# AlejandroSilvestri/os1

Hardware: AMD Instinct MI355X
Metric: frames/sec extract+match, 1920x1080 @ 2000 ORB feats (higher is better)
Workload: dtype u8

## Files before the change

os1_amd/csrc/orbfe_extractor.hip:

```cpp
#include <hip/hip_runtime.h>
#include <unistd.h>
#include <sched.h>

#include <algorithm>
#include <cctype>
#include <chrono>
#include <cmath>
#include <cstdarg>
#include <cstdio>
#include <cstdlib>
#include <cstring>
#include <memory>
#include <mutex>
#include <string>
#include <thread>
#include <vector>

#include "../../include/orbfe.h"
#include "glibc_sincosf.h"
#include "host_pool.h"
#include "orbfe_internal.h"
#include "quadtree.h"

namespace orbfe {
// ... 292 lines not shown
    Q.minTh = minTh;
    long long off = 0, slot = 0;
    int cellBase = 0;
    size_t tableBytes = 0;
    for (int l = 0; l < nlevels; l++) {
      LevelGeom& L = Q.lv[l];
      L.w = cv_round_f((float)c * isf[l]);
      L.h = cv_round_f((float)r * isf[l]);
      const float width = (float)((L.w - kEdge + 3) - (kEdge - 3));
      const float height = (float)((L.h - kEdge + 3) - (kEdge - 3));
      L.nCols = (int)(width / 30.f);
      L.nRows = (int)(height / 30.f);
      if (L.nCols < 1 || L.nRows < 1) {
        set_err("image %dx%d too small: level %d (%dx%d) has no FAST cell", c, r, l, L.w, L.h);
        return ORBFE_ERR_TOO_SMALL;
      }
      L.wCell = (int)std::ceil(width / L.nCols);
      L.hCell = (int)std::ceil(height / L.nRows);
      {
        const int nIni = (int)roundf(static_cast<float>(L.w - 2 * kBorder) / (L.h - 2 * kBorder));
        if (nIni < 1 || nIni > 4) qtOk = false;
        kpSum += std::max(nfeat[l] + 4, 4 * std::max(nIni, 4));
      }
      L.cellBase = cellBase;
      cellBase += L.nCols * L.nRows;
      L.slotCap = (((L.wCell + 1) / 2) * ((L.hCell + 1) / 2) + 3) & ~3;
      L.slotBase = slot;
      slot += (long long)L.nCols * L.nRows * L.slotCap;
      if (l >= 1) {
        L.pitch = (int)align_up(L.w, 64);
        L.off = off;
        off += align_up((long long)L.pitch * L.h, 256);
        tableBytes += align_up(L.w * 4, 16) + align_up(L.w * 4, 16) + align_up(L.h * 4, 16) + align_up(L.h * 4, 16) + align_up(L.h * 4, 16);
      }
    }
    Q.ncells = cellBase;
    Q.slabBytes = off;
    Q.slotsPerFrame = slot;
    Q.candCap = slot;
    if (slot >= (1ll << 24)) qtOk = false;

    std::vector<uint8_t> tab(tableBytes);
    int rc = d_tables.ensure(tableBytes);
    if (rc) return rc;
    size_t cur = 0;
    const int* xofsH[kMaxLevels] = {};
    const int* yofsH[kMaxLevels] = {};
    for (int l = 1; l < nlevels; l++) {
      LevelGeom& L = Q.lv[l];
      const int sw = Q.lv[l - 1].w, sh = Q.lv[l - 1].h, dw = L.w, dh = L.h;
      const double scale_x = 1. / ((double)dw / sw), scale_y = 1. / ((double)dh / sh);
      int* xofs = (int*)(tab.data() + cur);
      xofsH[l] = xofs;
      L.xofs = (const int*)(d_tables.p + cur);
      cur += align_up(dw * 4, 16);
      short* xa = (short*)(tab.data() + cur);
      L.xalpha = (const short*)(d_tables.p + cur);
      cur += align_up(dw * 4, 16);
      int* yofs = (int*)(tab.data() + cur);
      yofsH[l] = yofs;
      L.yofs = (const int*)(d_tables.p + cur);
      cur += align_up(dh * 4, 16);
      short* yb = (short*)(tab.data() + cur);
      L.ybeta = (const short*)(d_tables.p + cur);
      cur += align_up(dh * 4, 16);
      unsigned* yc = (unsigned*)(tab.data() + cur);
// ... 5 lines not shown
        fx -= sx;
        if (sx < 0) { fx = 0; sx = 0; }
        if (sx >= sw - 1) { fx = 0; sx = sw - 1; }
        xofs[dx] = sx;
        xa[2 * dx] = sat_short(cv_round_f((1.f - fx) * 2048));
        xa[2 * dx + 1] = sat_short(cv_round_f(fx * 2048));
      }
      for (int dy = 0; dy < dh; dy++) {
        float fy = (float)((dy + 0.5) * scale_y - 0.5);
        int sy = cv_floor_f(fy);
        fy -= sy;
        yofs[dy] = sy;
        yc[dy] = (unsigned)std::min(std::max(sy, 0), sh - 1) | ((unsigned)std::min(std::max(sy + 1, 0), sh - 1) << 16);
        yb[2 * dy] = sat_short(cv_round_f((1.f - fy) * 2048));
        yb[2 * dy + 1] = sat_short(cv_round_f(fy * 2048));
      }
      for (int dy = dh; dy < (int)align_up(dh, 4); dy++) {
        yc[dy] = yc[dh - 1];
        yb[2 * dy] = yb[2 * (dh - 1)];
        yb[2 * dy + 1] = yb[2 * (dh - 1) + 1];
      }
      int maxW = 1, maxH = 1;
      for (int x0 = 0; x0 < dw; x0 += 64) {
        const int x1 = std::min(x0 + 64, dw) - 1;
        maxW = std::max(maxW, std::min(xofs[x1] + 1, sw - 1) - xofs[x0] + 1);
      }
      for (int y0 = 0; y0 < dh; y0 += 64) {
        const int y1 = std::min(y0 + 64, dh) - 1;
        const int r0 = std::min(std::max(yofs[y0], 0), sh - 1), r1 = std::min(std::max(yofs[y1] + 1, 0), sh - 1);
        maxH = std::max(maxH, r1 - r0 + 1);
      }
      L.rzPitch = (maxW + 3 + 3) & ~3;
      L.rzRows = maxH;
    }
    HIP_TRY(hipMemcpyAsync(d_tables.p, tab.data(), tableBytes, hipMemcpyHostToDevice, stream));
    auto buildCone = [&](int tile, int baseMin, ConeParams& out, DevBuf<ConeRange>& tabBuf, bool& ok) -> int {
      ok = false;
      if (!(nlevels >= 3 && scaleFactor <= 1.5f)) return ORBFE_OK;
      std::vector<ConeRange> coneTab;
      const int top = nlevels - 1;
      if (tile <= 0) {
        tile = 32;
        for (int t = 16; t < 32; t += 2)
          if (((Q.lv[top].w + t - 1) / t) * ((Q.lv[top].h + t - 1) / t) <= 256) { tile = t; break; }
      }
      const int tx = (Q.lv[top].w + tile - 1) / tile, ty = (Q.lv[top].h + tile - 1) / tile;
      coneTab.assign((size_t)(tx + ty) * kMaxLevels, ConeRange{0, 0});
      int maxW[kMaxLevels] = {}, maxH[kMaxLevels] = {};
      for (int b = 0; b < tx + ty; b++) {
        const bool isX = b < tx;
        int lo = (isX ? b : b - tx) * tile, hi = std::min(lo + tile, isX ? Q.lv[top].w : Q.lv[top].h) - 1;
        ConeRange* R = coneTab.data() + (size_t)b * kMaxLevels;
        for (int l = top;; l--) {
          R[l] = ConeRange{lo, hi};
          int& m = isX ? maxW[l] : maxH[l];
          m = std::max(m, hi - lo + 1);
          if (l == 0) break;
          const int dn = isX ? Q.lv[l].w : Q.lv[l].h, sn = isX ? Q.lv[l - 1].w : Q.lv[l - 1].h;
          const int* ofs = isX ? xofsH[l] : yofsH[l];
          const int nlo = lo == 0 ? 0 : std::min(std::max(ofs[lo], 0), sn - 1);
          const int nhi = hi == dn - 1 ? sn - 1 : std::min(std::max(ofs[hi] + 1, 0), sn - 1);
          lo = nlo; hi = nhi;
        }
      }
      for (int base = std::max(0, baseMin); base < top - 1; base++) {
        auto pitchOf = [&](int l) { return (maxW[l] + 3 + 3) & ~3; };
// ... 1726 lines not shown
```

os1_amd/csrc/orbfe_internal.h:

```cpp
#pragma once
#include <cstddef>
#include <cstdint>

#include "equidistant_tan.h"

namespace orbfe {

constexpr int kMaxLevels = 12;
constexpr int kEdge = 19;
constexpr int kBorder = 16;
constexpr int kHalfPatch = 15;
constexpr int kBlurRad = 18;
constexpr int kRawRad = kBlurRad + 3;

struct LevelGeom {
  int w, h;
  int pitch;
  long long off;
  int nCols, nRows;
  int wCell, hCell;
  int cellBase;
  int slotCap;
  long long slotBase;
  const int* xofs;
  const short* xalpha;
  const int* yofs;
  const short* ybeta;
  const unsigned* yofc;
  int rzPitch, rzRows;
};

struct FastCell {
  uint16_t ex0, ey0;
  uint8_t ew, pad0;
  uint8_t eh, level;
  uint32_t cell;
  uint32_t slotOff;
  uint32_t roiOff;
  uint32_t pitch;
  uint8_t wCell, hCell;
  uint16_t pad1;
  uint32_t geo;
};
static_assert(sizeof(FastCell) == 32, "one s_load_dwordx8 per FAST wave");

struct PyramidParams {
  LevelGeom lv[kMaxLevels];
  int nlevels;
  int ncells;
  long long slabBytes;
  long long slotsPerFrame;
  long long candCap;
  const uint8_t* const* frame0;
  const uint8_t* frameInline[2];
  long long stride0;
  uint8_t* slab;
  uint32_t* cellCount;
  uint32_t* slots;
  uint32_t* cand;
  uint32_t* levelStart;
  const FastCell* cells;
  const uint8_t* zeros;
// ... 116 lines not shown
```

os1_amd/csrc/orbfe_kernels.hip:

```cpp
#include <mutex>
#include <hip/hip_runtime.h>

#include <type_traits>

#include "glibc_sincosf.h"
#include "orbfe_internal.h"

namespace orbfe {

__device__ __forceinline__ int m24(int a, int b) { return __mul24(a, b); }
__device__ __forceinline__ unsigned mulu24(unsigned a, unsigned b) {
  unsigned r;
  asm("v_mul_u32_u24 %0, %1, %2" : "=v"(r) : "v"(a), "v"(b));
  return r;
}

constexpr int kRzTile = 64;

__global__ __launch_bounds__(256) void k_resize(PyramidParams P, int level) {
  extern __shared__ __align__(16) uint8_t rz[];
  const LevelGeom& D = P.lv[level];
  const LevelGeom& S = P.lv[level - 1];
  const int f = P.frameBase + blockIdx.z;
  const int tx0 = blockIdx.x * kRzTile, ty0 = blockIdx.y * kRzTile;
  const int tx1 = min(tx0 + kRzTile, D.w) - 1, ty1 = min(ty0 + kRzTile, D.h) - 1;
  const uint8_t* src;
  long long sstride;
  if (level == 1) {
    src = level0_of(P, f);
    sstride = P.stride0;
  } else {
    src = P.slab + (long long)f * P.slabBytes + S.off;
// ... 84 lines not shown
}
__device__ __forceinline__ unsigned mulu24_w1(unsigned b, unsigned hh) {
  unsigned r;
  asm("v_mul_u32_u24_sdwa %0, %1, %2 dst_sel:DWORD dst_unused:UNUSED_PAD src0_sel:DWORD src1_sel:WORD_1" : "=v"(r) : "v"(b), "v"(hh));
  return r;
}

template <int WA, int WB>
__device__ __forceinline__ unsigned mulu24_hh(unsigned a, unsigned b) {
  unsigned r;
  if (WA == 0 && WB == 0) asm("v_mul_u32_u24_sdwa %0, %1, %2 dst_sel:DWORD dst_unused:UNUSED_PAD src0_sel:WORD_0 src1_sel:WORD_0" : "=v"(r) : "v"(a), "v"(b));
  if (WA == 0 && WB == 1) asm("v_mul_u32_u24_sdwa %0, %1, %2 dst_sel:DWORD dst_unused:UNUSED_PAD src0_sel:WORD_0 src1_sel:WORD_1" : "=v"(r) : "v"(a), "v"(b));
  if (WA == 1 && WB == 0) asm("v_mul_u32_u24_sdwa %0, %1, %2 dst_sel:DWORD dst_unused:UNUSED_PAD src0_sel:WORD_1 src1_sel:WORD_0" : "=v"(r) : "v"(a), "v"(b));
  if (WA == 1 && WB == 1) asm("v_mul_u32_u24_sdwa %0, %1, %2 dst_sel:DWORD dst_unused:UNUSED_PAD src0_sel:WORD_1 src1_sel:WORD_1" : "=v"(r) : "v"(a), "v"(b));
  return r;
}

__device__ __forceinline__ int ld32(const void* base, unsigned byteOff) {
  return *reinterpret_cast<const int*>(reinterpret_cast<const char*>(base) + byteOff);
}

__device__ __forceinline__ const uint8_t* uniform_ptr(const uint8_t* p) {
  const uintptr_t v = reinterpret_cast<uintptr_t>(p);
  const unsigned lo = __builtin_amdgcn_readfirstlane((unsigned)v), hi = __builtin_amdgcn_readfirstlane((unsigned)(v >> 32));
  return reinterpret_cast<const uint8_t*>(((uintptr_t)hi << 32) | lo);
}

__device__ __forceinline__ unsigned pk_round2(unsigned x, unsigned y) {
  unsigned t;
  asm("v_pk_add_u16 %0, %1, %2\n\tv_pk_add_u16 %0, %0, 2 op_sel_hi:[1,0]\n\tv_pk_lshrrev_b16 %0, 2, %0 op_sel_hi:[0,1]" : "=&v"(t) : "v"(x), "v"(y));
  return t;
}

struct ResizeLevel {
  int dw, dh, dpitch;
  int sw, sh;
  long long sstride;
  long long doff, soff;
  const int* xofs;
  const short* xalpha;
  const unsigned* yofc;
  const short* ybeta;
  const uint8_t* const* frame0;
  const uint8_t* frameInline[2];
  uint8_t* slab;
  long long slabBytes;
  int frameBase;
  int fromLevel0;
};

template <int LP, int RH>
__global__ __launch_bounds__(256) void k_resize_fixed(ResizeLevel R, int tilesX, int ntiles, unsigned rcpTilesX, int dma) {
  __shared__ __align__(16) uint8_t rz[LP * RH];
  __shared__ __align__(16) uint16_t H[RH * 64];
  struct { int w, h, pitch; const int* xofs; const short* xalpha; const unsigned* yofc; const short* ybeta; } D = {R.dw, R.dh, R.dpitch, R.xofs, R.xalpha, R.yofc, R.ybeta};
  struct { int w, h; } S = {R.sw, R.sh};
  const int f = R.frameBase + blockIdx.y;
  const int chunk = (ntiles + 7) >> 3;
  const int tileIx = (blockIdx.x & 7) * chunk + (blockIdx.x >> 3);
  if (tileIx >= ntiles) return;
  const int tyI = (int)(((unsigned long long)(unsigned)tileIx * rcpTilesX) >> 32);
  const int tx0 = (tileIx - tyI * tilesX) * kRzTile, ty0 = tyI * kRzTile;
  const int tx1 = min(tx0 + kRzTile, D.w) - 1, ty1 = min(ty0 + kRzTile, D.h) - 1;
  const int level = R.fromLevel0 ? 1 : 2;
  typedef uint32_t u32x2 __attribute__((ext_vector_type(2)));
  u32x2 fpw = {0u, 0u};
  if (R.fromLevel0) {
    if (R.frame0) {
      fpw = *reinterpret_cast<const u32x2 __attribute__((address_space(4)))*>(reinterpret_cast<uintptr_t>(R.frame0 + f));
    } else {
      const unsigned long long v = reinterpret_cast<unsigned long long>((f & 1) ? R.frameInline[1] : R.frameInline[0]);
      fpw.x = (uint32_t)v;
      fpw.y = (uint32_t)(v >> 32);
    }
  }
  const int cxa = *reinterpret_cast<const int __attribute__((address_space(4)))*>(reinterpret_cast<uintptr_t>(D.xofs + tx0));
  const int cxb = *reinterpret_cast<const int __attribute__((address_space(4)))*>(reinterpret_cast<uintptr_t>(D.xofs + tx1));
  const unsigned cya = *reinterpret_cast<const unsigned __attribute__((address_space(4)))*>(reinterpret_cast<uintptr_t>(D.yofc + ty0));
  const unsigned cyb = *reinterpret_cast<const unsigned __attribute__((address_space(4)))*>(reinterpret_cast<uintptr_t>(D.yofc + ty1));
  const int tid = threadIdx.x;
  const int hc = tid & 63;
  const int hx = min(tx0 + hc, D.w - 1);
  const int hsx = ld32(D.xofs, (unsigned)hx << 2);
  const int hal = ld32(D.xalpha, (unsigned)hx << 2);
  const int cx = tx0 + (tid & 15) * 4, cy = ty0 + (tid >> 4) * 4;
  const int4 syq = *reinterpret_cast<const int4*>(reinterpret_cast<const char*>(D.yofc) + ((unsigned)cy << 2));
  const int4 beq = *reinterpret_cast<const int4*>(reinterpret_cast<const char*>(D.ybeta) + ((unsigned)cy << 2));
  const int syv[4] = {syq.x, syq.y, syq.z, syq.w}, be[4] = {beq.x, beq.y, beq.z, beq.w};
  asm volatile("" ::"s"(cxa), "s"(cxb), "s"(cya), "s"(cyb), "s"(fpw.x), "s"(fpw.y));
  const uint8_t* src;
  const long long sstride = R.sstride;
  if (R.fromLevel0) {
    src = reinterpret_cast<const uint8_t*>(((unsigned long long)fpw.y << 32) | fpw.x);
  } else {
    src = R.slab + (long long)f * R.slabBytes + R.soff;
  }
  const int rx0 = cxa, rx1 = min(cxb + 1, S.w - 1);
  const int ry0 = (int)(cya & 0xffffu), ry1 = (int)(cyb >> 16);
  const int rw = rx1 - rx0 + 1, rh = ry1 - ry0 + 1;
  const int istr = (int)sstride;
  const uint8_t* rbase = uniform_ptr(src + (long long)ry0 * sstride + rx0);
  const int a = (int)(reinterpret_cast<uintptr_t>(rbase) & 3);
  if ((sstride & 3) == 0 && dma) {
    static_assert(LP == 96 && RH % 10 == 0, "LDS-DMA staging layout");
    const uint8_t* gb = rbase - a;
    const int lane = tid & 63, wave = __builtin_amdgcn_readfirstlane(tid >> 6);
    const int lrow = (int)(((unsigned)lane * 43u) >> 8), lcol = lane - lrow * 6;
    const bool lastSpecial = level == 1 && ry1 == S.h - 1;
    const int rhDma = lastSpecial ? rh - 1 : rh;
    const bool on = lrow < 10 && 16 * lcol < a + rw;
    const unsigned voff = (unsigned)(m24(lrow, istr) + 16 * lcol);
#pragma unroll
    for (int u = 0; u < RH / 40; u++) {
      const int r = (wave * (RH / 40) + u) * 10;
      const uint8_t* gbr = gb + (long long)r * sstride;
      unsigned vo = voff;
      asm volatile("" : "+s"(gbr), "+v"(vo));
      if (on && r + lrow < rhDma)
        __builtin_amdgcn_global_load_lds((const __attribute__((address_space(1))) void*)(gbr + vo),
                                         (__attribute__((address_space(3))) void*)(rz + r * LP), 16, 0, 0);
    }
    if (lastSpecial && tid < ((a + rw + 3) >> 2))
      *reinterpret_cast<uint32_t*>(rz + (rh - 1) * LP + 4 * tid) = (uint32_t)ld32(gb, (unsigned)(4 * tid + m24(rh - 1, istr)));
    asm volatile("s_waitcnt vmcnt(0)" ::: "memory");
  } else if ((sstride & 3) == 0) {
    static_assert(LP <= 128 && RH % 8 == 0, "staging layout");
    const int ndw = (a + rw + 3) >> 2;
    const int c = tid & 31, r0 = tid >> 5;
    if (c < ndw) {
      const uint8_t* gb = rbase - a;
      uint32_t v[RH / 8];
#pragma unroll
      for (int u = 0; u < RH / 8; u++) v[u] = (uint32_t)ld32(gb, (unsigned)(4 * c + m24(min(r0 + 8 * u, rh - 1), istr)));
      uint8_t* l = rz + 4 * c + r0 * LP;
#pragma unroll
      for (int u = 0; u < RH / 8; u++) *reinterpret_cast<uint32_t*>(l + u * 8 * LP) = v[u];
    }
  } else {
    const float rcp = 1.0f / (float)rw;
    const int total = rw * rh;
    for (int i = tid; i < total; i += 256) {
      const int y = (int)(((float)i + 0.5f) * rcp), x = i - m24(y, rw);
      rz[y * LP + a + x] = rbase[m24(y, istr) + x];
    }
  }
  __syncthreads();
  {
    const unsigned a0 = (unsigned)(int)(short)hal << 12, a1 = (unsigned)(hal >> 16) << 12;
    const int o0 = a + hsx - rx0, o1 = a + min(hsx + 1, S.w - 1) - rx0;
    const uint8_t* p0 = rz + (tid >> 6) * LP + o0;
    const uint8_t* p1 = rz + (tid >> 6) * LP + o1;
    uint16_t* h = H + (tid >> 6) * 64 + hc;
#pragma unroll
    for (int i = 0; i < RH / 4; i++)
      h[i * 4 * 64] = (uint16_t)((__umul24(p0[i * 4 * LP], a0) + __umul24(p1[i * 4 * LP], a1)) >> 16);
  }
  __syncthreads();
  if (cx > tx1 || cy > ty1) return;
  uint8_t* dst = R.slab + (long long)f * R.slabBytes + R.doff;
  unsigned doffs = (unsigned)(m24(cy, D.pitch) + cx);
  const unsigned hx2 = (unsigned)(cx - tx0) * 2u, ry0s = (unsigned)ry0 << 7;
#pragma unroll
  for (int j = 0; j < 4; j++) {
    const int y = cy + j;
    if (y > ty1) break;
    const unsigned r0 = ((unsigned)syv[j] & 0xffffu) << 7, r1 = ((unsigned)syv[j] >> 16) << 7;
    const uint8_t* hb = reinterpret_cast<const uint8_t*>(H) + hx2 - ry0s;
    const uint2 q0 = *reinterpret_cast<const uint2*>(hb + r0), q1 = *reinterpret_cast<const uint2*>(hb + r1);
    const unsigned bw = (unsigned)be[j];
    const unsigned x01 = __builtin_amdgcn_perm(mulu24_hh<0, 1>(bw, q0.x), mulu24_hh<0, 0>(bw, q0.x), 0x07060302u);
    const unsigned y01 = __builtin_amdgcn_perm(mulu24_hh<1, 1>(bw, q1.x), mulu24_hh<1, 0>(bw, q1.x), 0x07060302u);
    const unsigned x23 = __builtin_amdgcn_perm(mulu24_hh<0, 1>(bw, q0.y), mulu24_hh<0, 0>(bw, q0.y), 0x07060302u);
    const unsigned y23 = __builtin_amdgcn_perm(mulu24_hh<1, 1>(bw, q1.y), mulu24_hh<1, 0>(bw, q1.y), 0x07060302u);
    const unsigned v01 = pk_round2(x01, y01), v23 = pk_round2(x23, y23);
    *reinterpret_cast<uint32_t*>(dst + doffs) = __builtin_amdgcn_perm(v23, v01, 0x06040200u);
    doffs += (unsigned)D.pitch;
  }
}

constexpr int kConeThreads = 1024;
#ifdef ORBFE_EXPERIMENTS
__device__ unsigned long long g_coneStamps[32];
#define CONE_STAMP(i)                                                                                                              \
  do {                                                                                                                             \
    if (threadIdx.x == 0 && blockIdx.z == 0 && blockIdx.x == gridDim.x / 2 && blockIdx.y == gridDim.y / 2)                         \
      g_coneStamps[i] = __builtin_amdgcn_s_memrealtime();                                                                          \
  } while (0)
#else
#define CONE_STAMP(i) ((void)0)
#endif

__global__ __launch_bounds__(kConeThreads) void k_pyramid_cone(PyramidParams P, ConeParams C) {
  extern __shared__ __align__(16) uint8_t cone[];
  const int tid = threadIdx.x, f = P.frameBase + blockIdx.z;
// ... 431 lines not shown
  if constexpr (w2 != 0u) acc = __builtin_amdgcn_udot4(d[2], w2, acc, false);
  if constexpr (w3 != 0u) acc = __builtin_amdgcn_udot4(d[3], w3, acc, false);
  return acc;
}

__device__ __forceinline__ int wave_sum_i32(int v) {
  v += __builtin_amdgcn_update_dpp(v, v, 0x128, 0xf, 0xf, false);
  v += __builtin_amdgcn_update_dpp(v, v, 0x124, 0xf, 0xf, false);
  v += __builtin_amdgcn_update_dpp(v, v, 0x122, 0xf, 0xf, false);
  v += __builtin_amdgcn_update_dpp(v, v, 0x121, 0xf, 0xf, false);
  return __builtin_amdgcn_readlane(v, 0) + __builtin_amdgcn_readlane(v, 16) + __builtin_amdgcn_readlane(v, 32) +
         __builtin_amdgcn_readlane(v, 48);
}

__device__ __forceinline__ void wave_sum3_i32(int& a, int& b, int& c) {
#define ORBFE_ROR3(n)                                                          \
  "v_add_u32_dpp %0, %0, %0 row_ror:" #n " row_mask:0xf bank_mask:0xf\n\t"     \
  "v_add_u32_dpp %1, %1, %1 row_ror:" #n " row_mask:0xf bank_mask:0xf\n\t"     \
  "v_add_u32_dpp %2, %2, %2 row_ror:" #n " row_mask:0xf bank_mask:0xf\n\t"
  asm volatile("s_nop 1\n\t" ORBFE_ROR3(8) ORBFE_ROR3(4) ORBFE_ROR3(2) ORBFE_ROR3(1) : "+v"(a), "+v"(b), "+v"(c));
#undef ORBFE_ROR3
  a = __builtin_amdgcn_readlane(a, 0) + __builtin_amdgcn_readlane(a, 16) + __builtin_amdgcn_readlane(a, 32) + __builtin_amdgcn_readlane(a, 48);
  b = __builtin_amdgcn_readlane(b, 0) + __builtin_amdgcn_readlane(b, 16) + __builtin_amdgcn_readlane(b, 32) + __builtin_amdgcn_readlane(b, 48);
  c = __builtin_amdgcn_readlane(c, 0) + __builtin_amdgcn_readlane(c, 16) + __builtin_amdgcn_readlane(c, 32) + __builtin_amdgcn_readlane(c, 48);
}

struct SlotInfo {
  const uint32_t* selCount;
  int selPerFrame;
  int selOff[kMaxLevels + 1];
  int nlevels;
};

struct DescribeLevel { int w, h, pitch, pad; long long off, pad2; };
struct DescribeArgs {
  DescribeLevel lv[kMaxLevels];
  const SelKp* sel;
  const uint32_t* selCount;
  float* angleOut;
  uint8_t* descOut;
  float* angleOut2;
  uint8_t* descOut2;
  const uint8_t* const* frame0;
  const uint8_t* frameInline[2];
  long long stride0;
  uint8_t* slab;
  long long slabBytes;
  int nsel, selPerFrame, nlevels, frameBase, dma;
  int selOff[kMaxLevels + 1];
  int gauss;
};

template <int WAVES, int GAUSS>
__global__ __launch_bounds__(64 * WAVES) void k_describe(DescribeArgs A) {
  constexpr int NT = 64 * WAVES;
  constexpr int NIC = (kIcItems + NT - 1) / NT, NH = (kBlurItemsHost.nh + NT - 1) / NT, NV = (kBlurItemsHost.nv + NT - 1) / NT;
  static_assert(NIC * NT <= 256 && NH * NT <= 512 && NV <= NH, "table padding");
  uint32_t icw[NIC][3], bh[NH], bv[NV];
#pragma unroll
  for (int it = 0; it < NIC; it++) {
    const IcW w = c_icTab.e[it * NT + threadIdx.x];
    icw[it][0] = w.w1; icw[it][1] = w.w2; icw[it][2] = w.w3;
  }
#pragma unroll
  for (int it = 0; it < NH; it++) bh[it] = c_blurCodes.h[it * NT + threadIdx.x];
#pragma unroll
  for (int it = 0; it < NV; it++) bv[it] = c_blurCodes.v[it * NT + threadIdx.x];
  __shared__ int icSum[3 * WAVES];
  __shared__ __align__(16) uint8_t raw[kRawW * kRawP + 16];
  __shared__ __align__(16) uint16_t hbT[40 * kHPT];
  static_assert(kBlurW * kBPT <= kRawW * kRawP, "the blurred patch must fit into the raw patch");
  uint8_t* blT = raw;
  asm volatile("" ::"s"(A.sel), "s"(A.selCount), "s"(A.angleOut), "s"(A.descOut), "s"(A.frame0), "s"(A.frameInline[0]), "s"(A.frameInline[1]),
               "s"(A.stride0), "s"(A.slab), "s"(A.slabBytes), "s"(A.nsel), "s"(A.selPerFrame), "s"(A.nlevels), "s"(A.frameBase), "s"(A.dma),
               "s"(A.selOff[1]), "s"(A.selOff[2]), "s"(A.selOff[3]), "s"(A.selOff[4]), "s"(A.selOff[5]), "s"(A.selOff[6]), "s"(A.selOff[7]));
  const int nsel = A.nsel, dma = A.dma;
  const SelKp* sel = A.sel;
  float* angleOut = A.angleOut;
  uint8_t* descOut = A.descOut;
  const int chunk = (nsel + 7) >> 3;
  const int k = (blockIdx.x & 7) * chunk + (blockIdx.x >> 3);
  if (k >= nsel) return;
  const int tid = threadIdx.x, lane = tid & 63, wave = WAVES == 1 ? 0 : __builtin_amdgcn_readfirstlane(tid >> 6);
  typedef uint32_t u32x2 __attribute__((ext_vector_type(2)));
  typedef uint32_t u32x8 __attribute__((ext_vector_type(8)));
  const char __attribute__((address_space(4)))* ka = (const char __attribute__((address_space(4)))*)__builtin_amdgcn_kernarg_segment_ptr();
  int level, f;
  u32x2 sw, fpw = {0u, 0u};
  u32x8 lw;
  auto frame_ptr_words = [&](int fa) -> u32x2 {
    u32x2 r;
    if (A.frame0) {
      r = *reinterpret_cast<const u32x2 __attribute__((address_space(4)))*>(reinterpret_cast<uintptr_t>(A.frame0 + fa));
    } else {
      const unsigned long long v = reinterpret_cast<unsigned long long>((fa & 1) ? A.frameInline[1] : A.frameInline[0]);
      r.x = (uint32_t)v;
      r.y = (uint32_t)(v >> 32);
    }
    return r;
  };
  if (A.selCount) {
    const int fr = k / A.selPerFrame, within = k - fr * A.selPerFrame;
    int l = 0, lbase = 0;
#pragma unroll
    for (int j = 1; j < kMaxLevels; j++) {
      const int o = A.selOff[j];
      if (j < A.nlevels && within >= o) { l = j; lbase = o; }
    }
    level = l;
    f = A.frameBase + fr;
    const uint32_t live = *reinterpret_cast<const uint32_t __attribute__((address_space(4)))*>(
        reinterpret_cast<uintptr_t>(A.selCount + (long long)f * kMaxLevels + l));
    sw = *reinterpret_cast<const u32x2 __attribute__((address_space(4)))*>(reinterpret_cast<uintptr_t>(sel + k));
    fpw = frame_ptr_words(f);
    lw = *reinterpret_cast<const u32x8 __attribute__((address_space(4)))*>(ka + offsetof(DescribeArgs, lv) + 32 * (unsigned)l);
    asm volatile("" ::"s"(sw.x), "s"(live), "s"(fpw.x), "s"(lw[0]));
    if ((uint32_t)(within - lbase) >= live) return;
  } else {
    sw = *reinterpret_cast<const u32x2 __attribute__((address_space(4)))*>(reinterpret_cast<uintptr_t>(sel + k));
    level = (int)(sw.y & 0xffu);
    f = (int)((sw.y >> 8) & 0xffffu);
    fpw = frame_ptr_words(f);
    lw = *reinterpret_cast<const u32x8 __attribute__((address_space(4)))*>(ka + offsetof(DescribeArgs, lv) + 32 * (unsigned)level);
  }
  const int cx = (int)(sw.x & 0xffffu), cy = (int)(sw.x >> 16);
  struct { int w, h; } L = {(int)lw[0], (int)lw[1]};
  const uint8_t* img;
  long long stride;
  if (level == 0) {
    img = reinterpret_cast<const uint8_t*>(((unsigned long long)fpw.y << 32) | fpw.x);
    stride = A.stride0;
  } else {
    img = A.slab + (long long)f * A.slabBytes + (long long)(((unsigned long long)lw[5] << 32) | lw[4]);
    stride = (long long)(int)lw[2];
  }
  int pa = 0;
  const int istr = (int)stride;
  const bool interior = cx >= kRawRad && cy >= kRawRad && cx + kRawRad < L.w && cy + kRawRad < L.h && (stride & 3) == 0;
  if (interior && dma && (level != 0 || cy + kRawRad < L.h - 1)) {
    const uint8_t* rbase = uniform_ptr(img + m24(cy - kRawRad, istr) + (cx - kRawRad));
    pa = (int)(reinterpret_cast<uintptr_t>(rbase) & 3);
    const uint8_t* gb = rbase - pa;
    constexpr int RPI = WAVES == 1 ? 21 : 11, NI = WAVES == 1 ? 3 : 1;
    static_assert(RPI * NI * WAVES >= kRawW && 3 * RPI <= 64 && kRawP == 48, "LDS-DMA patch layout");
    const int lrow = (lane * 171) >> 9, lcol = lane - 3 * lrow;
    const unsigned voff = (unsigned)(m24(lrow, istr) + 16 * lcol);
#pragma unroll
    for (int u = 0; u < NI; u++) {
      const int r = (wave * NI + u) * RPI;
      if (lrow < RPI && r + lrow < kRawW)
// ... 252 lines not shown
    if (ok[u]) *reinterpret_cast<T*>(dst + dof[u]) = v[u];
}

void launch_ingest(const uint8_t* src, long long sstride, uint8_t* dst, long long dpitch, int rowBytes, int rows, hipStream_t st) {
  const uintptr_t all = (uintptr_t)src | (uintptr_t)dst | (uintptr_t)sstride | (uintptr_t)dpitch | (uintptr_t)rowBytes;
  const int V = (all & 15) == 0 ? 16 : (all & 3) == 0 ? 4 : 1;
  constexpr int U = 4;
  const long long total = (long long)((rowBytes + V - 1) / V) * rows;
  const int blocks = (int)std::max<long long>(1, (total + 256 * U - 1) / (256 * U));
#define ORBFE_INGEST(VV, UU) hipLaunchKernelGGL((k_ingest<VV, UU>), dim3(blocks), dim3(256), 0, st, src, sstride, dst, dpitch, rowBytes, rows)
  if (V == 16) ORBFE_INGEST(16, 4);
  else if (V == 4) ORBFE_INGEST(4, 4);
  else ORBFE_INGEST(1, 4);
#undef ORBFE_INGEST
}

int launch_pyramid(const PyramidParams& P, int nframes, hipStream_t st, const ConeParams* cone) {
  const int last = cone ? cone->base : P.nlevels - 1;
  if (cone) {
    static std::mutex mu;
    static int attrBytes[64] = {};
    int dev = 0;
    if (hipGetDevice(&dev) != hipSuccess || dev < 0 || dev >= 64) return 1;
    std::lock_guard<std::mutex> lk(mu);
    if (cone->ldsBytes > attrBytes[dev]) {
      if (hipFuncSetAttribute(reinterpret_cast<const void*>(k_pyramid_cone), hipFuncAttributeMaxDynamicSharedMemorySize,
                              cone->ldsBytes) != hipSuccess)
        return 1;
      attrBytes[dev] = cone->ldsBytes;
    }
  }
  for (int l = 1; l <= last; l++) {
    dim3 grid((P.lv[l].w + kRzTile - 1) / kRzTile, (P.lv[l].h + kRzTile - 1) / kRzTile, nframes);
    if (P.lv[l].rzPitch <= 96 && P.lv[l].rzRows <= 80 && grid.x >= 2) {
      const int tilesX = (int)grid.x, ntiles = (int)(grid.x * grid.y);
      const unsigned rcp = (unsigned)(0x100000000ull / (unsigned)tilesX) + 1u;
      if ((unsigned long long)ntiles * tilesX < (1ull << 31)) {
        const int dma = lds_dma_enabled();
        ResizeLevel R{};
        R.dw = P.lv[l].w; R.dh = P.lv[l].h; R.dpitch = P.lv[l].pitch;
        R.sw = P.lv[l - 1].w; R.sh = P.lv[l - 1].h;
        R.sstride = l == 1 ? P.stride0 : (long long)P.lv[l - 1].pitch;
        R.doff = P.lv[l].off; R.soff = P.lv[l - 1].off;
        R.xofs = P.lv[l].xofs; R.xalpha = P.lv[l].xalpha; R.yofc = P.lv[l].yofc; R.ybeta = P.lv[l].ybeta;
        R.frame0 = P.frame0; R.frameInline[0] = P.frameInline[0]; R.frameInline[1] = P.frameInline[1];
        R.slab = P.slab; R.slabBytes = P.slabBytes; R.frameBase = P.frameBase; R.fromLevel0 = l == 1;
        hipLaunchKernelGGL((k_resize_fixed<96, 80>), dim3(8 * ((ntiles + 7) / 8), nframes), dim3(256), 0, st, R, tilesX, ntiles, rcp, dma);
        continue;
      }
    }
    hipLaunchKernelGGL(k_resize, grid, dim3(256), (((size_t)P.lv[l].rzPitch * P.lv[l].rzRows + 15) & ~(size_t)15) + (size_t)P.lv[l].rzRows * 64 * 2, st,
                       P, l);
  }
  if (cone)
    hipLaunchKernelGGL(k_pyramid_cone, dim3(cone->tilesX, cone->tilesY, nframes), dim3(kConeThreads), cone->ldsBytes, st, P, *cone);
  return 0;
}

void launch_compact(const PyramidParams& P, int nframes, hipStream_t st) {
  hipLaunchKernelGGL(k_compact, dim3((P.ncells + 63) / 64, nframes), dim3(64), 0, st, P);
}
void launch_compact_local(const PyramidParams& P, int nframes, hipStream_t st, int level0, int level1) {
  if (level1 > P.nlevels) level1 = P.nlevels;
  int maxCells = 0;
  for (int l = level0; l < level1; l++) maxCells = std::max(maxCells, P.lv[l].nCols * P.lv[l].nRows);
  if (maxCells <= 0) return;
  hipLaunchKernelGGL(k_compact_local, dim3((maxCells + 63) / 64, level1 - level0, nframes), dim3(64), 0, st, P, level0);
}

static DescribeArgs describe_args(const PyramidParams& P, const SelKp* sel, int nsel, float* angle, uint8_t* desc) {
  DescribeArgs A{};
  for (int l = 0; l < kMaxLevels; l++) {
    A.lv[l].w = P.lv[l].w; A.lv[l].h = P.lv[l].h; A.lv[l].pitch = P.lv[l].pitch; A.lv[l].off = P.lv[l].off;
  }
  A.sel = sel; A.selCount = nullptr; A.angleOut = angle; A.descOut = desc; A.angleOut2 = nullptr; A.descOut2 = nullptr;
  A.frame0 = P.frame0; A.frameInline[0] = P.frameInline[0]; A.frameInline[1] = P.frameInline[1];
  A.stride0 = P.stride0; A.slab = P.slab; A.slabBytes = P.slabBytes;
  A.nsel = nsel; A.selPerFrame = 1; A.nlevels = P.nlevels; A.frameBase = P.frameBase; A.dma = lds_dma_enabled();
  A.gauss = P.gaussVariant;
  return A;
}

void launch_describe(const PyramidParams& P, const SelKp* sel, int nsel, float* angle, uint8_t* desc,
                     hipStream_t st) {
  if (nsel <= 0) return;
  const DescribeArgs A = describe_args(P, sel, nsel, angle, desc);
  if (A.gauss == 1) hipLaunchKernelGGL((k_describe<1, 1>), dim3(8 * ((nsel + 7) / 8)), dim3(64), 0, st, A);
  else hipLaunchKernelGGL((k_describe<1, 0>), dim3(8 * ((nsel + 7) / 8)), dim3(64), 0, st, A);
}

void launch_describe_slots(const PyramidParams& P, const SelKp* sel, int nslots, float* angle, uint8_t* desc,
                           const uint32_t* selCount, int selPerFrame, const int* selOff, hipStream_t st, bool fourWaves, float* angle2,
                           uint8_t* desc2) {
  if (nslots <= 0) return;
  DescribeArgs A = describe_args(P, sel, nslots, angle, desc);
  A.angleOut2 = angle2;
  A.descOut2 = desc2;
  A.selCount = selCount;
  A.selPerFrame = selPerFrame;
  for (int l = 0; l <= P.nlevels; l++) A.selOff[l] = selOff[l];
  const dim3 grid(8 * ((nslots + 7) / 8));
  if (fourWaves) {
    if (A.gauss == 1) hipLaunchKernelGGL((k_describe<4, 1>), grid, dim3(256), 0, st, A);
    else hipLaunchKernelGGL((k_describe<4, 0>), grid, dim3(256), 0, st, A);
  } else {
    if (A.gauss == 1) hipLaunchKernelGGL((k_describe<1, 1>), grid, dim3(64), 0, st, A);
    else hipLaunchKernelGGL((k_describe<1, 0>), grid, dim3(64), 0, st, A);
  }
}

__global__ void k_spin(unsigned long long ticks, unsigned* sink) {
  const unsigned long long t0 = __builtin_amdgcn_s_memrealtime();
  unsigned n = 0;
  while (__builtin_amdgcn_s_memrealtime() - t0 < ticks) { __builtin_amdgcn_s_sleep(32); n++; }
  if (sink && n == 0xffffffffu) *sink = n;
}
void launch_spin(unsigned long long ticks, hipStream_t st) {
  hipLaunchKernelGGL(k_spin, dim3(1), dim3(64), 0, st, ticks, (unsigned*)nullptr);
}

void launch_sincos(const float* deg, int n, float* c, float* s, hipStream_t st) {
  if (n <= 0) return;
  hipLaunchKernelGGL(k_sincos, dim3((n + 255) / 256), dim3(256), 0, st, deg, n, c, s);
}

}

#ifdef ORBFE_EXPERIMENTS
extern "C" int orbfe_exp_cone_stamps(unsigned long long* out ) {
  if (hipDeviceSynchronize() != hipSuccess) return 1;
  return hipMemcpyFromSymbol(out, HIP_SYMBOL(orbfe::g_coneStamps), sizeof(unsigned long long) * 32) == hipSuccess ? 0 : 1;
}
#endif
// ... 1 lines not shown
```

Baseline: 90040.

## Precompute resize tile records on host and specialize resize kernel staging

Per-tile geometry for the fixed resize kernel (tile bounds, source window, offsets, DMA row counts) is now computed once on the host into 64-byte records uploaded with the level tables. Each block reads its record with one scalar load instead of doing division and table lookups. The staging mode becomes a template parameter so the runtime branch is removed. Describe also gets a reciprocal-multiply frame index and a scalar compare chain for level lookup, with per-level selOff stored in the level struct. These trim scalar prologue work in small kernels, at the cost of more table memory and more kernel instantiations.

```diff
diff --git a/os1_amd/csrc/orbfe_extractor.hip b/os1_amd/csrc/orbfe_extractor.hip
--- a/os1_amd/csrc/orbfe_extractor.hip
+++ b/os1_amd/csrc/orbfe_extractor.hip
@@ -348,6 +348,7 @@
         L.off = off;
         off += align_up((long long)L.pitch * L.h, 256);
         tableBytes += align_up(L.w * 4, 16) + align_up(L.w * 4, 16) + align_up(L.h * 4, 16) + align_up(L.h * 4, 16) + align_up(L.h * 4, 16);
+        tableBytes += 64 + sizeof(ResizeTile) * (size_t)resize_tile_blocks(L.w, L.h);
       }
     }
     Q.ncells = cellBase;
@@ -419,6 +420,19 @@
       }
       L.rzPitch = (maxW + 3 + 3) & ~3;
       L.rzRows = maxH;
+      L.tiles = nullptr;
+      L.tileBlocks = 0;
+      cur = align_up(cur, 64);
+      if (L.rzPitch <= 96 && L.rzRows <= 80 && resize_tiles_x(dw) >= 2) {
+        ResizeTileLevel T{dw, dh, L.pitch, sw, sh, L.off, Q.lv[l - 1].off, l == 1, xofs, yc};
+        std::vector<ResizeTile> recs;
+        if (build_resize_tiles(T, recs)) {
+          memcpy(tab.data() + cur, recs.data(), sizeof(ResizeTile) * recs.size());
+          L.tiles = (const ResizeTile*)(d_tables.p + cur);
+          L.tileBlocks = (int)recs.size();
+        }
+      }
+      cur += sizeof(ResizeTile) * (size_t)resize_tile_blocks(dw, dh);
     }
     HIP_TRY(hipMemcpyAsync(d_tables.p, tab.data(), tableBytes, hipMemcpyHostToDevice, stream));
     auto buildCone = [&](int tile, int baseMin, ConeParams& out, DevBuf<ConeRange>& tabBuf, bool& ok) -> int {
diff --git a/os1_amd/csrc/orbfe_internal.h b/os1_amd/csrc/orbfe_internal.h
--- a/os1_amd/csrc/orbfe_internal.h
+++ b/os1_amd/csrc/orbfe_internal.h
@@ -3,6 +3,7 @@
 #include <cstdint>
 
 #include "equidistant_tan.h"
+#include "resize_tiles.h"
 
 namespace orbfe {
 
@@ -28,6 +29,8 @@
   const short* ybeta;
   const unsigned* yofc;
   int rzPitch, rzRows;
+  const ResizeTile* tiles;
+  int tileBlocks;
 };
 
 struct FastCell {
diff --git a/os1_amd/csrc/orbfe_kernels.hip b/os1_amd/csrc/orbfe_kernels.hip
--- a/os1_amd/csrc/orbfe_kernels.hip
+++ b/os1_amd/csrc/orbfe_kernels.hip
@@ -1,3 +1,4 @@
+#include <climits>
 #include <mutex>
 #include <hip/hip_runtime.h>
 
@@ -148,11 +149,12 @@
   return t;
 }
 
+enum { kStageDma = 0, kStageDwords = 1, kStageBytes = 2 };
 struct ResizeLevel {
-  int dw, dh, dpitch;
-  int sw, sh;
-  long long sstride;
-  long long doff, soff;
+  int dpitch;
+  int sw;
+  int sstride;
+  const ResizeTile* tiles;
   const int* xofs;
   const short* xalpha;
   const unsigned* yofc;
@@ -165,21 +167,17 @@
   int fromLevel0;
 };
 
-template <int LP, int RH>
-__global__ __launch_bounds__(256) void k_resize_fixed(ResizeLevel R, int tilesX, int ntiles, unsigned rcpTilesX, int dma) {
+template <int LP, int RH, int STAGE>
+__global__ __launch_bounds__(256) void k_resize_fixed(ResizeLevel R) {
   __shared__ __align__(16) uint8_t rz[LP * RH];
   __shared__ __align__(16) uint16_t H[RH * 64];
-  struct { int w, h, pitch; const int* xofs; const short* xalpha; const unsigned* yofc; const short* ybeta; } D = {R.dw, R.dh, R.dpitch, R.xofs, R.xalpha, R.yofc, R.ybeta};
-  struct { int w, h; } S = {R.sw, R.sh};
+  struct { int pitch; const int* xofs; const short* xalpha; const unsigned* yofc; const short* ybeta; } D = {R.dpitch, R.xofs, R.xalpha, R.yofc, R.ybeta};
+  struct { int w; } S = {R.sw};
   const int f = R.frameBase + blockIdx.y;
-  const int chunk = (ntiles + 7) >> 3;
-  const int tileIx = (blockIdx.x & 7) * chunk + (blockIdx.x >> 3);
-  if (tileIx >= ntiles) return;
-  const int tyI = (int)(((unsigned long long)(unsigned)tileIx * rcpTilesX) >> 32);
-  const int tx0 = (tileIx - tyI * tilesX) * kRzTile, ty0 = tyI * kRzTile;
-  const int tx1 = min(tx0 + kRzTile, D.w) - 1, ty1 = min(ty0 + kRzTile, D.h) - 1;
-  const int level = R.fromLevel0 ? 1 : 2;
   typedef uint32_t u32x2 __attribute__((ext_vector_type(2)));
+  typedef uint32_t u32x16 __attribute__((ext_vector_type(16)));
+  static_assert(kRzTile == kRzTileEdge, "tile edge of the records");
+  const u32x16 tw = *reinterpret_cast<const u32x16 __attribute__((address_space(4)))*>(reinterpret_cast<uintptr_t>(R.tiles + blockIdx.x));
   u32x2 fpw = {0u, 0u};
   if (R.fromLevel0) {
     if (R.frame0) {
@@ -190,46 +188,41 @@
       fpw.y = (uint32_t)(v >> 32);
     }
   }
-  const int cxa = *reinterpret_cast<const int __attribute__((address_space(4)))*>(reinterpret_cast<uintptr_t>(D.xofs + tx0));
-  const int cxb = *reinterpret_cast<const int __attribute__((address_space(4)))*>(reinterpret_cast<uintptr_t>(D.xofs + tx1));
-  const unsigned cya = *reinterpret_cast<const unsigned __attribute__((address_space(4)))*>(reinterpret_cast<uintptr_t>(D.yofc + ty0));
-  const unsigned cyb = *reinterpret_cast<const unsigned __attribute__((address_space(4)))*>(reinterpret_cast<uintptr_t>(D.yofc + ty1));
+  asm volatile("" ::"s"(tw[0]), "s"(fpw.x), "s"(fpw.y));
+  const int tx0 = (int)tw[2], ty0 = (int)tw[3], tx1 = (int)tw[4], ty1 = (int)tw[5];
+  const int rx0 = (int)tw[6], ry0 = (int)tw[7], rw = (int)tw[8], rh = (int)tw[9];
+  if (rh == 0) return;
   const int tid = threadIdx.x;
   const int hc = tid & 63;
-  const int hx = min(tx0 + hc, D.w - 1);
+  const int hx = min(tx0 + hc, tx1);
   const int hsx = ld32(D.xofs, (unsigned)hx << 2);
   const int hal = ld32(D.xalpha, (unsigned)hx << 2);
   const int cx = tx0 + (tid & 15) * 4, cy = ty0 + (tid >> 4) * 4;
   const int4 syq = *reinterpret_cast<const int4*>(reinterpret_cast<const char*>(D.yofc) + ((unsigned)cy << 2));
   const int4 beq = *reinterpret_cast<const int4*>(reinterpret_cast<const char*>(D.ybeta) + ((unsigned)cy << 2));
   const int syv[4] = {syq.x, syq.y, syq.z, syq.w}, be[4] = {beq.x, beq.y, beq.z, beq.w};
-  asm volatile("" ::"s"(cxa), "s"(cxb), "s"(cya), "s"(cyb), "s"(fpw.x), "s"(fpw.y));
   const uint8_t* src;
-  const long long sstride = R.sstride;
   if (R.fromLevel0) {
     src = reinterpret_cast<const uint8_t*>(((unsigned long long)fpw.y << 32) | fpw.x);
   } else {
-    src = R.slab + (long long)f * R.slabBytes + R.soff;
-  }
-  const int rx0 = cxa, rx1 = min(cxb + 1, S.w - 1);
-  const int ry0 = (int)(cya & 0xffffu), ry1 = (int)(cyb >> 16);
-  const int rw = rx1 - rx0 + 1, rh = ry1 - ry0 + 1;
-  const int istr = (int)sstride;
-  const uint8_t* rbase = uniform_ptr(src + (long long)ry0 * sstride + rx0);
+    src = R.slab + (long long)f * R.slabBytes;
+  }
+  const int istr = R.sstride;
+  const uint8_t* rbase = uniform_ptr(src + (tw[0] + (unsigned)ry0 * (unsigned)istr));
   const int a = (int)(reinterpret_cast<uintptr_t>(rbase) & 3);
-  if ((sstride & 3) == 0 && dma) {
+  if constexpr (STAGE == kStageDma) {
     static_assert(LP == 96 && RH % 10 == 0, "LDS-DMA staging layout");
     const uint8_t* gb = rbase - a;
     const int lane = tid & 63, wave = __builtin_amdgcn_readfirstlane(tid >> 6);
     const int lrow = (int)(((unsigned)lane * 43u) >> 8), lcol = lane - lrow * 6;
-    const bool lastSpecial = level == 1 && ry1 == S.h - 1;
-    const int rhDma = lastSpecial ? rh - 1 : rh;
+    const bool lastSpecial = tw[11] != 0u;
+    const int rhDma = (int)tw[10];
     const bool on = lrow < 10 && 16 * lcol < a + rw;
     const unsigned voff = (unsigned)(m24(lrow, istr) + 16 * lcol);
 #pragma unroll
     for (int u = 0; u < RH / 40; u++) {
       const int r = (wave * (RH / 40) + u) * 10;
-      const uint8_t* gbr = gb + (long long)r * sstride;
+      const uint8_t* gbr = gb + (unsigned)r * (unsigned)istr;
       unsigned vo = voff;
       asm volatile("" : "+s"(gbr), "+v"(vo));
       if (on && r + lrow < rhDma)
@@ -239,7 +232,7 @@
     if (lastSpecial && tid < ((a + rw + 3) >> 2))
       *reinterpret_cast<uint32_t*>(rz + (rh - 1) * LP + 4 * tid) = (uint32_t)ld32(gb, (unsigned)(4 * tid + m24(rh - 1, istr)));
     asm volatile("s_waitcnt vmcnt(0)" ::: "memory");
-  } else if ((sstride & 3) == 0) {
+  } else if constexpr (STAGE == kStageDwords) {
     static_assert(LP <= 128 && RH % 8 == 0, "staging layout");
     const int ndw = (a + rw + 3) >> 2;
     const int c = tid & 31, r0 = tid >> 5;
@@ -273,9 +266,9 @@
   }
   __syncthreads();
   if (cx > tx1 || cy > ty1) return;
-  uint8_t* dst = R.slab + (long long)f * R.slabBytes + R.doff;
-  unsigned doffs = (unsigned)(m24(cy, D.pitch) + cx);
-  const unsigned hx2 = (unsigned)(cx - tx0) * 2u, ry0s = (unsigned)ry0 << 7;
+  uint8_t* dst = R.slab + (long long)f * R.slabBytes + tw[1];
+  unsigned doffs = (unsigned)(m24((tid >> 4) * 4, D.pitch) + (tid & 15) * 4);
+  const unsigned hx2 = (unsigned)(tid & 15) * 8u, ry0s = (unsigned)ry0 << 7;
 #pragma unroll
   for (int j = 0; j < 4; j++) {
     const int y = cy + j;
@@ -773,7 +766,7 @@
   int nlevels;
 };
 
-struct DescribeLevel { int w, h, pitch, pad; long long off, pad2; };
+struct DescribeLevel { int w, h, pitch, selOff; long long off, pad2; };
 struct DescribeArgs {
   DescribeLevel lv[kMaxLevels];
   const SelKp* sel;
@@ -789,6 +782,7 @@
   long long slabBytes;
   int nsel, selPerFrame, nlevels, frameBase, dma;
   int selOff[kMaxLevels + 1];
+  unsigned rcpSelPerFrame;
   int gauss;
 };
 
@@ -814,7 +808,8 @@
   uint8_t* blT = raw;
   asm volatile("" ::"s"(A.sel), "s"(A.selCount), "s"(A.angleOut), "s"(A.descOut), "s"(A.frame0), "s"(A.frameInline[0]), "s"(A.frameInline[1]),
                "s"(A.stride0), "s"(A.slab), "s"(A.slabBytes), "s"(A.nsel), "s"(A.selPerFrame), "s"(A.nlevels), "s"(A.frameBase), "s"(A.dma),
-               "s"(A.selOff[1]), "s"(A.selOff[2]), "s"(A.selOff[3]), "s"(A.selOff[4]), "s"(A.selOff[5]), "s"(A.selOff[6]), "s"(A.selOff[7]));
+               "s"(A.selOff[1]), "s"(A.selOff[2]), "s"(A.selOff[3]), "s"(A.selOff[4]), "s"(A.selOff[5]), "s"(A.selOff[6]), "s"(A.selOff[7]),
+               "s"(A.selOff[8]), "s"(A.selOff[9]), "s"(A.selOff[10]), "s"(A.selOff[11]), "s"(A.rcpSelPerFrame));
   const int nsel = A.nsel, dma = A.dma;
   const SelKp* sel = A.sel;
   float* angleOut = A.angleOut;
@@ -841,13 +836,11 @@
     return r;
   };
   if (A.selCount) {
-    const int fr = k / A.selPerFrame, within = k - fr * A.selPerFrame;
-    int l = 0, lbase = 0;
-#pragma unroll
-    for (int j = 1; j < kMaxLevels; j++) {
-      const int o = A.selOff[j];
-      if (j < A.nlevels && within >= o) { l = j; lbase = o; }
-    }
+    const int fr = A.rcpSelPerFrame ? (int)__umulhi((unsigned)k, A.rcpSelPerFrame) : k / A.selPerFrame;
+    const int within = k - fr * A.selPerFrame;
+    int l = 0;
+#pragma unroll
+    for (int j = 1; j < kMaxLevels; j++) asm("s_cmp_ge_i32 %1, %2\n\ts_addc_u32 %0, %0, 0" : "+s"(l) : "s"(within), "s"(A.selOff[j]) : "scc");
     level = l;
     f = A.frameBase + fr;
     const uint32_t live = *reinterpret_cast<const uint32_t __attribute__((address_space(4)))*>(
@@ -856,7 +849,7 @@
     fpw = frame_ptr_words(f);
     lw = *reinterpret_cast<const u32x8 __attribute__((address_space(4)))*>(ka + offsetof(DescribeArgs, lv) + 32 * (unsigned)l);
     asm volatile("" ::"s"(sw.x), "s"(live), "s"(fpw.x), "s"(lw[0]));
-    if ((uint32_t)(within - lbase) >= live) return;
+    if ((uint32_t)(within - (int)lw[3]) >= live) return;
   } else {
     sw = *reinterpret_cast<const u32x2 __attribute__((address_space(4)))*>(reinterpret_cast<uintptr_t>(sel + k));
     level = (int)(sw.y & 0xffu);
@@ -1175,22 +1168,18 @@
   }
   for (int l = 1; l <= last; l++) {
     dim3 grid((P.lv[l].w + kRzTile - 1) / kRzTile, (P.lv[l].h + kRzTile - 1) / kRzTile, nframes);
-    if (P.lv[l].rzPitch <= 96 && P.lv[l].rzRows <= 80 && grid.x >= 2) {
-      const int tilesX = (int)grid.x, ntiles = (int)(grid.x * grid.y);
-      const unsigned rcp = (unsigned)(0x100000000ull / (unsigned)tilesX) + 1u;
-      if ((unsigned long long)ntiles * tilesX < (1ull << 31)) {
-        const int dma = lds_dma_enabled();
-        ResizeLevel R{};
-        R.dw = P.lv[l].w; R.dh = P.lv[l].h; R.dpitch = P.lv[l].pitch;
-        R.sw = P.lv[l - 1].w; R.sh = P.lv[l - 1].h;
-        R.sstride = l == 1 ? P.stride0 : (long long)P.lv[l - 1].pitch;
-        R.doff = P.lv[l].off; R.soff = P.lv[l - 1].off;
-        R.xofs = P.lv[l].xofs; R.xalpha = P.lv[l].xalpha; R.yofc = P.lv[l].yofc; R.ybeta = P.lv[l].ybeta;
-        R.frame0 = P.frame0; R.frameInline[0] = P.frameInline[0]; R.frameInline[1] = P.frameInline[1];
-        R.slab = P.slab; R.slabBytes = P.slabBytes; R.frameBase = P.frameBase; R.fromLevel0 = l == 1;
-        hipLaunchKernelGGL((k_resize_fixed<96, 80>), dim3(8 * ((ntiles + 7) / 8), nframes), dim3(256), 0, st, R, tilesX, ntiles, rcp, dma);
-        continue;
-      }
+    const long long sstride = l == 1 ? P.stride0 : (long long)P.lv[l - 1].pitch;
+    if (P.lv[l].tiles && sstride > 0 && (long long)P.lv[l - 1].h * sstride < (1ll << 31)) {
+      ResizeLevel R{};
+      R.dpitch = P.lv[l].pitch; R.sw = P.lv[l - 1].w; R.sstride = (int)sstride; R.tiles = P.lv[l].tiles;
+      R.xofs = P.lv[l].xofs; R.xalpha = P.lv[l].xalpha; R.yofc = P.lv[l].yofc; R.ybeta = P.lv[l].ybeta;
+      R.frame0 = P.frame0; R.frameInline[0] = P.frameInline[0]; R.frameInline[1] = P.frameInline[1];
+      R.slab = P.slab; R.slabBytes = P.slabBytes; R.frameBase = P.frameBase; R.fromLevel0 = l == 1;
+      const dim3 tgrid(P.lv[l].tileBlocks, nframes);
+      if ((sstride & 3) != 0) hipLaunchKernelGGL((k_resize_fixed<96, 80, kStageBytes>), tgrid, dim3(256), 0, st, R);
+      else if (lds_dma_enabled()) hipLaunchKernelGGL((k_resize_fixed<96, 80, kStageDma>), tgrid, dim3(256), 0, st, R);
+      else hipLaunchKernelGGL((k_resize_fixed<96, 80, kStageDwords>), tgrid, dim3(256), 0, st, R);
+      continue;
     }
     hipLaunchKernelGGL(k_resize, grid, dim3(256), (((size_t)P.lv[l].rzPitch * P.lv[l].rzRows + 15) & ~(size_t)15) + (size_t)P.lv[l].rzRows * 64 * 2, st,
                        P, l);
@@ -1241,7 +1230,10 @@
   A.descOut2 = desc2;
   A.selCount = selCount;
   A.selPerFrame = selPerFrame;
-  for (int l = 0; l <= P.nlevels; l++) A.selOff[l] = selOff[l];
+  for (int l = 0; l <= kMaxLevels; l++) A.selOff[l] = l < P.nlevels ? selOff[l] : INT_MAX;
+  for (int l = 0; l < P.nlevels; l++) A.lv[l].selOff = selOff[l];
+  if (selPerFrame >= 2 && (unsigned long long)nslots * (unsigned long long)selPerFrame < (1ull << 32))
+    A.rcpSelPerFrame = (unsigned)(0x100000000ull / (unsigned)selPerFrame) + 1u;
   const dim3 grid(8 * ((nslots + 7) / 8));
   if (fourWaves) {
     if (A.gauss == 1) hipLaunchKernelGGL((k_describe<4, 1>), grid, dim3(256), 0, st, A);
diff --git a/os1_amd/csrc/resize_tiles.h b/os1_amd/csrc/resize_tiles.h
--- /dev/null
+++ b/os1_amd/csrc/resize_tiles.h
@@ -0,0 +1,69 @@
+#pragma once
+#include <algorithm>
+#include <cstdint>
+#include <vector>
+
+namespace orbfe {
+
+constexpr int kRzTileEdge = 64;
+
+struct ResizeTile {
+  uint32_t srcOff;
+  uint32_t dstOff;
+  int32_t tx0, ty0;
+  int32_t tx1, ty1;
+  int32_t rx0, ry0;
+  int32_t rw, rh;
+  int32_t rhDma;
+  int32_t lastSpecial;
+  int32_t pad[4];
+};
+static_assert(sizeof(ResizeTile) == 64, "one s_load_dwordx16 per block");
+
+struct ResizeTileLevel {
+  int dw, dh, dpitch;
+  int sw, sh;
+  long long doff, soff;
+  bool fromLevel0;
+  const int* xofs;
+  const unsigned* yofc;
+};
+
+inline int resize_tiles_x(int dw) { return (dw + kRzTileEdge - 1) / kRzTileEdge; }
+inline int resize_tiles_y(int dh) { return (dh + kRzTileEdge - 1) / kRzTileEdge; }
+inline int resize_tile_blocks(int dw, int dh) { return 8 * ((resize_tiles_x(dw) * resize_tiles_y(dh) + 7) / 8); }
+
+inline bool build_resize_tiles(const ResizeTileLevel& L, std::vector<ResizeTile>& out) {
+  const int tilesX = resize_tiles_x(L.dw), ntiles = tilesX * resize_tiles_y(L.dh), chunk = (ntiles + 7) / 8;
+  out.assign((size_t)8 * chunk, ResizeTile{});
+  for (int b = 0; b < 8 * chunk; b++) {
+    const int tile = (b & 7) * chunk + (b >> 3);
+    if (tile >= ntiles) continue;
+    ResizeTile& t = out[b];
+    t.tx0 = (tile % tilesX) * kRzTileEdge;
+    t.ty0 = (tile / tilesX) * kRzTileEdge;
+    t.tx1 = std::min(t.tx0 + kRzTileEdge, L.dw) - 1;
+    t.ty1 = std::min(t.ty0 + kRzTileEdge, L.dh) - 1;
+    t.rx0 = L.xofs[t.tx0];
+    const int rx1 = std::min(L.xofs[t.tx1] + 1, L.sw - 1);
+    t.ry0 = (int)(L.yofc[t.ty0] & 0xffffu);
+    const int ry1 = (int)(L.yofc[t.ty1] >> 16);
+    t.rw = rx1 - t.rx0 + 1;
+    t.rh = ry1 - t.ry0 + 1;
+    t.lastSpecial = L.fromLevel0 && ry1 == L.sh - 1;
+    t.rhDma = t.lastSpecial ? t.rh - 1 : t.rh;
+    const long long so = (L.fromLevel0 ? 0 : L.soff) + t.rx0;
+    const long long dO = L.doff + (long long)t.ty0 * L.dpitch + t.tx0;
+    if (so < 0 || so >= (1ll << 32) || dO < 0 || dO >= (1ll << 32) || t.rw <= 0 || t.rh <= 0) return false;
+    t.srcOff = (uint32_t)so;
+    t.dstOff = (uint32_t)dO;
+  }
+  return true;
+}
+
+inline uint32_t resize_tile_first_byte(const ResizeTile& t, uint32_t stride) { return t.srcOff + (uint32_t)t.ry0 * stride; }
+inline int resize_tile_align(const ResizeTile& t, uintptr_t srcBase, uint32_t stride) {
+  return (int)((srcBase + resize_tile_first_byte(t, stride)) & 3);
+}
+
+}
```

After: 90870, median of 6. About the same (+0.9%).
